# lxm0851/mp3

Measured on AMD Instinct MI355X. Metric: stereo MP3 frames/s (128 kbps 44.1 kHz) at 1/2/4/8 GPU; % HBM roofline, higher is better.
Workload: dtype f32; 1 GPU; C3: full Layer III decode (Huffman->PCM), 65536 streams x 32 frames per GPU per step; streams_per_gpu=65536, hz=44100, seed=default, parallelism=streams sharded, 1 process per GPU, no data-path collective

## Files before the change

mp3_amd/csrc/mp3d_huffman.hip:

```cpp
#include <algorithm>

#include "mp3d_huffman_dev.h"

namespace mp3d {

#define RANK_BINS 320
#define RANK_BLOCK 1024
#define RANK_PER 4
#define RANK_SEG (RANK_BLOCK * RANK_PER)
__global__ void __launch_bounds__(RANK_BLOCK) k_rank(const uint64_t *__restrict__ sideu, int n_units,
                                                     uint32_t *__restrict__ perm) {
    __shared__ uint32_t h[RANK_BINS];
    MP3D_LDS_ENTRY();
    const int tid = threadIdx.x, seg0 = blockIdx.x * RANK_SEG;
    for (int i = tid; i < RANK_BINS; i += RANK_BLOCK) h[i] = 0u;
    __syncthreads();
    uint32_t bin[RANK_PER], r[RANK_PER];
#pragma unroll
    for (int j = 0; j < RANK_PER; j++) {
        const int u = seg0 + j * RANK_BLOCK + tid;
        const uint32_t bv = u < n_units ? (uint32_t)(sideu[u] >> 43) & 0x1FFu : 0u;
        bin[j] = RANK_BINS - 1u - (bv < RANK_BINS ? bv : RANK_BINS - 1u);
        r[j] = u < n_units ? atomicAdd(&h[bin[j]], 1u) : 0u;
    }
    __syncthreads();
    if (tid < 64) {
        uint32_t c[5], sum = 0u;
#pragma unroll
        for (int k = 0; k < 5; k++) {
            c[k] = h[5 * tid + k];
            sum += c[k];
        }
        const uint32_t incl = wave_incl_scan(sum);
        uint32_t run = incl - sum;
#pragma unroll
        for (int k = 0; k < 5; k++) {
            h[5 * tid + k] = run;
            run += c[k];
        }
    }
    __syncthreads();
#pragma unroll
    for (int j = 0; j < RANK_PER; j++) {
        const int u = seg0 + j * RANK_BLOCK + tid;
        if (u < n_units) perm[seg0 + h[bin[j]] + r[j]] = (uint32_t)u;
    }
}

__global__ void __launch_bounds__(HUFF_BLOCK) k_huffman(const uint8_t *__restrict__ md, const uint64_t *__restrict__ md_off,
                                                        const FrameRec *__restrict__ rec,
                                                        const uint64_t *__restrict__ sideu,
                                                        const DevTables *__restrict__ tab, int16_t *__restrict__ is_buf,
                                                        UnitMeta *__restrict__ meta, int n_units, int F,
                                                        uint32_t *__restrict__ work, const uint32_t *__restrict__ perm) {
    __shared__ __attribute__((aligned(16))) uint16_t s_lut[MP3D_LUT_MAX];
    __shared__ __attribute__((aligned(16))) uint32_t s_bits[4 + HUFF_WAVES * (HUFF_CAPW + 4)];
    __shared__ uint32_t s_tsel[32];
    __shared__ uint16_t s_lbnd[9][24];
    __shared__ uint8_t s_slen[32];
    __shared__ uint32_t s_c1s[256];
    MP3D_LDS_ENTRY();
    huff_tables_lane(tab, s_lut, s_tsel, s_lbnd, s_slen);
    static_assert(HUFF_BLOCK >= 256, "s_c1s: one entry per thread");
    if (threadIdx.x < 256) {
        const uint32_t v = threadIdx.x >> 4, s4 = threadIdx.x & 15u;
        int q[4], j = 0;
#pragma unroll
        for (int i = 0; i < 4; i++) {
            const int bit = (int)(v >> (3 - i)) & 1;
            q[i] = bit && ((s4 >> (3 - j)) & 1u) ? -1 : bit;
            j += bit;
        }
        s_c1s[threadIdx.x] = (uint32_t)(uint8_t)q[2] | (uint32_t)(uint8_t)q[0] << 8 | (uint32_t)(uint8_t)q[3] << 16 |
                             (uint32_t)(uint8_t)q[1] << 24;
    }
    __syncthreads();
    const int lane = threadIdx.x & 63, wv = threadIdx.x >> 6;
    uint32_t *bits = s_bits + 4 + wv * (HUFF_CAPW + 4);
    const uint32_t qbase = tab->lut_hdr.base[MP3D_LUT_TABLES - 1];
    const int qb1 = tab->lut_hdr.bits1[MP3D_LUT_TABLES - 1];
    const uint32_t c1b_base = ((qbase + (1u << qb1) + 1u) & ~1u) + MP3D_C1B_OFF;
    for (;;) {
        uint32_t t = 0u;
        if (lane == 0) t = atomicAdd(work, 1u);
        const int ubase = 64 * (int)__builtin_amdgcn_readfirstlane(t);
        if (ubase >= n_units) break;
        {
            const int u = ubase + lane < n_units ? (int)perm[ubase + lane] : n_units;
            const int fr = u >> 2, gr = (u >> 1) & 1, ch = u & 1;
            bool valid = u < n_units;
            const uint64_t mdo = md_off[(valid ? fr : 0) / F];
            FrameRec r;
            uint64_t sq[4] = {0, 0, 0, 0};
            if (valid) {
                r = rec[fr];
                valid = r.frame_bytes && !(r.first_gr & (REC_TAG | REC_DROP)) && ch < r.nch && (gr == 0 || !r.lsf);
                const ulonglong2 a = *(const ulonglong2 *)&sideu[u & ~3];
                const ulonglong2 b = *(const ulonglong2 *)&sideu[(u & ~3) + 2];
                sq[0] = a.x; sq[1] = a.y; sq[2] = b.x; sq[3] = b.y;
            }
            const int first_gr = valid ? (r.first_gr & 3) : 0;
            const int nch = valid ? r.nch : 1;
            const bool dec = valid && gr >= first_gr;
            const int q = u & 3;
            const uint64_t side = sq[q];
            const uint32_t p23 = dec ? (uint32_t)(side >> 52) : 0u;
            uint32_t before = 0;
#pragma unroll
            for (int qq = 0; qq < 3; qq++)
                if (qq < q && (qq >> 1) >= first_gr && (qq & 1) < nch) before += (uint32_t)(sq[qq] >> 52);
            const uint32_t start = dec ? r.md_bit + before : 0u;
            const int scfsi_raw = (int)(side >> 1) & 15;
            const bool long_blk = !(((side >> 30) & 1) && ((side >> 28) & 3) == 2);
            const int scfsi = (gr == 1 && long_blk) ? scfsi_raw : 0;
            const bool need_g0 = dec && scfsi && first_gr == 0;
            const uint32_t g0_start = r.md_bit + (ch ? (uint32_t)(sq[0] >> 52) : 0u);
            const uint32_t lenA = need_g0 ? HUFF_G0W : 0u;
            const uint32_t w0 = start >> 5;
            const uint32_t dA = need_g0 ? w0 - (g0_start >> 5) : 0u;
            const uint32_t lenB = dec ? ((((start + p23 + 31) >> 5) + 2 - w0 + 3) & ~3u) : 0u;
            const uint32_t len = lenA + lenB;
            const uint32_t incl = wave_incl_scan(len);
            const uint32_t off = incl - len;
            const uint32_t *src = (const uint32_t *)(md + (dec ? mdo : 0)) + w0;

            bool pending = dec;
            while (__ballot(pending)) {
                const uint32_t base = wave_min(pending ? off : 0xFFFFFFFFu);
                const bool inb = pending && off + len - base <= HUFF_STAGEW;
                wave_sync();
                if (inb) {
                    uint32_t *dst = bits + (off - base);
                    for (uint32_t i = 0; i < len; i += 16) {
                        uint4 v[4];
#pragma unroll
                        for (int k = 0; k < 4; k++) {
                            const uint32_t q = i + 4 * k;
                            if (q < len) v[k] = *(const uint4 *)(src + (int)(q < lenA ? q - dA : q - lenA));
                        }
#pragma unroll
                        for (int k = 0; k < 4; k++)
                            if (i + 4 * k < len)
                                *(uint4 *)(dst + i + 4 * k) =
                                    make_uint4(bswap32(v[k].x), bswap32(v[k].y), bswap32(v[k].z), bswap32(v[k].w));
                    }
                }
                wave_sync();
                if (inb) {
                    const uint32_t seg = 32u * (off - base + lenA) - 32u * w0;
                    uint32_t pos = start + seg;
                    int lsf_pre = 0;
                    if (r.lsf) {
                        const uint32_t pp = read_sf_lsf((lds_cu32)bits, pos, side, (uint8_t *)&meta[u]);
                        pos = pp & 0x7FFFFFFFu;
                        lsf_pre = (int)(pp >> 31);
                    } else {
                        uint32_t sfw[10];
#pragma unroll
                        for (int i = 0; i < 10; i++) sfw[i] = 0u;
                        if (need_g0) {
                            read_sf(bits, g0_start + seg - 32u * (lenA - dA), sq[ch], 0, sfw, s_slen);
                        }
                        pos = read_sf(bits, pos, side, scfsi, sfw, s_slen);
                        uint8_t *mrec = (uint8_t *)&meta[u];
                        *(uint4 *)mrec = make_uint4(sfw[0], sfw[1], sfw[2], sfw[3]);
                        *(uint4 *)(mrec + 16) = make_uint4(sfw[4], sfw[5], sfw[6], sfw[7]);
                        *(uint2 *)(mrec + 32) = make_uint2(sfw[8], sfw[9]);
                    }
                    const int ws = (int)(side >> 30) & 1;
                    const int bv2 = 2 * ((int)(side >> 43) & 0x1FF);
                    int r1, r2;
                    uint32_t ts0, ts1, ts2;
                    if (ws) {
                        const bool sh = ((side >> 28) & 3) == 2;
                        r1 = r.sr_idx < 3 ? 36 : sh ? (r.sr_idx == 8 ? 72 : 36) : (r.sr_idx == 8 ? 108 : 54);
                        r2 = 576;
                        ts0 = s_tsel[(side >> 22) & 31];
                        ts1 = s_tsel[(side >> 17) & 31];
                        ts2 = ts1;
                    } else {
                        const int rc0 = (int)(side >> 11) & 15, rc1 = (int)(side >> 8) & 7;
                        const int b1 = rc0 + 1;
                        int b2 = rc0 + rc1 + 2;
                        if (b2 > 22) b2 = 22;
                        r1 = s_lbnd[r.sr_idx][b1];
                        r2 = s_lbnd[r.sr_idx][b2];
                        ts0 = s_tsel[(side >> 25) & 31];
                        ts1 = s_tsel[(side >> 20) & 31];
                        ts2 = s_tsel[(side >> 15) & 31];
                    }
                    r1 = r1 < bv2 ? r1 : bv2;
                    r2 = r2 < bv2 ? r2 : bv2;
                    int16_t *row = is_buf + (size_t)u * MP3D_IS_ROW;
                    int k = 0;
                    const uint32_t end_bit = start + seg + p23;
                    uint4 pend = make_uint4(0u, 0u, 0u, 0u);
                    bool held = false;
                    for (; __ballot(k < bv2); k += 8) {
                        uint32_t wv[4];
#pragma unroll
                        for (int j = 0; j < 4; j++) {
                            const int kk = k + 2 * j;
                            const uint32_t ts = kk < r1 ? ts0 : (kk < r2 ? ts1 : ts2);
                            const uint32_t tb = ts & 0xFFFFu, s1 = (ts >> 16) & 63u, lin = ts >> 24;
                            uint32_t hi, lo;
                            win64g(bits, pos, hi, lo);
                            const uint32_t i1 = tb + (hi >> s1);
                            const uint32_t e1 = s_lut[i1];
                            const uint32_t nb = __builtin_amdgcn_ubfe(e1, 11, 4);
                            uint32_t b11 = __builtin_amdgcn_ubfe(e1, 0, 11);
                            __asm__("" : "+v"(b11));
                            const uint32_t sub = (b11 << 2) + __builtin_amdgcn_ubfe(hi, s1 - nb, nb);
                            const uint32_t i2 = (e1 & 0x8000u) ? sub : i1;
                            const uint32_t e = s_lut[i2];
                            const uint32_t x = (e >> 4) & 15u, y = e & 15u, len_c = (e >> 8) & 31u;
                            const uint32_t sx = (e >> 13) & 1u, sy = (e >> 14) & 1u;
                            const uint32_t rb = shl64hi_a(hi, lo, len_c);
                            const uint32_t nx = x == 15u ? lin : 0u, ny = y == 15u ? lin : 0u;
                            const uint32_t t0 = 32u - nx, t1 = t0 - sx, t2 = t1 - ny, t3 = t2 - sy;
                            const uint32_t ex = __builtin_amdgcn_ubfe(rb, t0, nx);
                            const uint32_t ey = __builtin_amdgcn_ubfe(rb, t2, ny);
                            const int mx = __builtin_amdgcn_sbfe((int)rb, t1, 1u), my = __builtin_amdgcn_sbfe((int)rb, t3, 1u);
                            const bool live = kk < bv2 && pos < end_bit;
                            pos += live ? len_c + (32u - t3) : 0u;
                            const int X = ((int)(x + ex) ^ mx) - mx, Y = ((int)(y + ey) ^ my) - my;
                            wv[j] = live ? __builtin_amdgcn_perm((uint32_t)Y, (uint32_t)X, 0x05040100u) : 0u;
                        }
                        const uint4 cur = make_uint4(wv[0], wv[1], wv[2], wv[3]);
                        if (held) {
                            *(uint4 *)(row + k - 8) = pend;
                            *(uint4 *)(row + k) = cur;
                        } else {
                            pend = cur;
                        }
                        held = !held;
                    }
                    if (held) *(uint4 *)(row + k - 8) = pend;
                    k = bv2;
                    const bool c1b = (side >> 5) & 1;
                    const uint32_t c1base = c1b ? c1b_base : qbase, c1sh = c1b ? 28u : 32u - (uint32_t)qb1;
                    auto c1_store = [&](int kq, uint32_t se) {
                        *(uint2 *)(row + kq) = make_uint2(__builtin_amdgcn_perm(se, se, 0x09030801u),
                                                          __builtin_amdgcn_perm(se << 8, se, 0x0B070A05u));
                    };
                    auto c1_dec = [&](uint32_t hw, uint32_t &se, uint32_t &nb) {
                        const uint32_t e = s_lut[c1base + (hw >> c1sh)];
                        const uint32_t v = e & 15u, lq = (e >> 8) & 31u;
                        nb = lq + __builtin_popcount(v);
                        se = s_c1s[(v << 4) | ((hw << lq) >> 28)];
                    };
                    while (k <= 572 && pos < end_bit) {
                        const uint32_t hw = win32g(bits, pos);
                        uint32_t se0, n0, se1, n1;
                        c1_dec(hw, se0, n0);
                        if (pos + n0 > end_bit) break;
                        pos += n0;
                        bool two = k <= 568 && pos < end_bit;
                        if (two) {
                            c1_dec(hw << n0, se1, n1);
                            two = pos + n1 <= end_bit;
                        }
                        if (!two) {
                            c1_store(k, se0);
                            k += 4;
                            break;
                        }
                        pos += n1;
                        const uint4 q = make_uint4(
                            __builtin_amdgcn_perm(se0, se0, 0x09030801u), __builtin_amdgcn_perm(se0 << 8, se0, 0x0B070A05u),
                            __builtin_amdgcn_perm(se1, se1, 0x09030801u), __builtin_amdgcn_perm(se1 << 8, se1, 0x0B070A05u));
                        __builtin_memcpy(row + k, &q, 16);
                        k += 8;
                    }
                    const int nz_end = k;
                    UnitMeta m;
                    m.global_gain = (uint8_t)(side >> 35);
                    m.block_type = (uint8_t)(ws ? (side >> 28) & 3 : 0);
                    m.mixed = (uint8_t)(ws && ((side >> 28) & 3) == 2 ? (side >> 27) & 1 : 0);
                    m.scalefac_scale = (uint8_t)((side >> 6) & 1);
                    m.preflag = (uint8_t)(r.lsf ? lsf_pre : (int)((side >> 7) & 1));
                    m.sbg[0] = (uint8_t)(ws ? (side >> 14) & 7 : 0);
                    m.sbg[1] = (uint8_t)(ws ? (side >> 11) & 7 : 0);
                    m.sbg[2] = (uint8_t)(ws ? (side >> 8) & 7 : 0);
                    m.nz_end = (uint16_t)nz_end;
                    m.part2_3_length = (uint16_t)p23;
                    m.used_bits = (uint16_t)(pos - start - seg);
                    m.flags = (uint16_t)(r.lsf ? ((side >> 31) & 1) << 1 : 0);
                    *(uint4 *)((uint8_t *)&meta[u] + 40) = *(const uint4 *)((const uint8_t *)&m + 40);
                }
                pending = pending && !inb;
            }
            if (valid && !dec) {
                int16_t *out = is_buf + (size_t)u * MP3D_IS_ROW;
                for (int kk = 0; kk < 576; kk += 8) *(uint4 *)(out + kk) = make_uint4(0, 0, 0, 0);
                UnitMeta m;
#pragma unroll
                for (int i = 0; i < 10; i++) ((uint32_t *)m.sf)[i] = 0u;
                const int ws = (int)(side >> 30) & 1;
                m.global_gain = (uint8_t)(side >> 35);
                m.block_type = (uint8_t)(ws ? (side >> 28) & 3 : 0);
                m.mixed = (uint8_t)(ws && ((side >> 28) & 3) == 2 ? (side >> 27) & 1 : 0);
                m.scalefac_scale = (uint8_t)((side >> 6) & 1);
                m.preflag = (uint8_t)(r.lsf ? 0 : (int)((side >> 7) & 1));
                m.sbg[0] = (uint8_t)(ws ? (side >> 14) & 7 : 0);
                m.sbg[1] = (uint8_t)(ws ? (side >> 11) & 7 : 0);
                m.sbg[2] = (uint8_t)(ws ? (side >> 8) & 7 : 0);
                m.nz_end = 0;
                m.part2_3_length = 0;
                m.used_bits = 0;
                m.flags = (uint16_t)(1 | (r.lsf ? ((side >> 31) & 1) << 1 : 0));
                meta[u] = m;
            }
        }
    }
}

__global__ void __launch_bounds__(64 * HW_UNITS) k_huffman_wave(const uint8_t *__restrict__ md,
                                                              const uint64_t *__restrict__ md_off,
                                                              const FrameRec *__restrict__ rec,
                                                              const uint64_t *__restrict__ sideu,
                                                              const DevTables *__restrict__ tab,
                                                              int16_t *__restrict__ is_buf,
                                                              UnitMeta *__restrict__ meta, int n_units, int F) {
    __shared__ __attribute__((aligned(16))) uint16_t s_lut[MP3D_LUT_MAX];
    __shared__ __attribute__((aligned(16))) uint32_t s_bits[HW_UNITS][HW_WORDS + 4];
    __shared__ uint32_t s_tsel[32];
    __shared__ uint16_t s_lbnd[9][24];
    __shared__ uint8_t s_slen[32];
    MP3D_LDS_ENTRY();
    huff_tables<64 * HW_UNITS>(tab, s_lut, s_tsel, s_lbnd, s_slen, threadIdx.x);
    __syncthreads();
    const int lane = threadIdx.x & 63;
    const int wv = __builtin_amdgcn_readfirstlane((int)(threadIdx.x >> 6));
    const int u = blockIdx.x * HW_UNITS + wv;
    if (u >= n_units) return;
    huffman_wave_unit(md, md_off, rec, sideu, tab, is_buf, meta, F, u, lane, s_bits[wv], s_lut, s_tsel, s_lbnd, s_slen);
}

void launch_huffman(const uint8_t *md, const uint64_t *md_off, const FrameRec *rec, const uint64_t *sideu,
                    const DevTables *tab, int16_t *is_buf, UnitMeta *meta, int n_streams, int F, int n_cu, bool wave,
                    uint32_t *work, uint32_t *rank, hipStream_t strm) {
    int n_units = n_streams * F * 4;
    if (wave) {
        hipLaunchKernelGGL(k_huffman_wave, dim3((n_units + HW_UNITS - 1) / HW_UNITS), dim3(64 * HW_UNITS), 0, strm, md,
                           md_off, rec, sideu, tab, is_buf, meta, n_units, F);
        return;
    }
    const int rounds = (n_units + 63) / 64;
    int blocks = (rounds + HUFF_WAVES - 1) / HUFF_WAVES;
    const int cus = n_cu > 0 ? n_cu : 256;
    blocks = blocks < cus ? (blocks > 0 ? blocks : 1) : cus;
    (void)hipMemsetAsync(work, 0, sizeof(uint32_t), strm);
    hipLaunchKernelGGL(k_rank, dim3((n_units + RANK_SEG - 1) / RANK_SEG), dim3(RANK_BLOCK), 0, strm, sideu, n_units, rank);
    hipLaunchKernelGGL(k_huffman, dim3(blocks), dim3(HUFF_BLOCK), 0, strm, md, md_off, rec, sideu, tab, is_buf, meta,
                       n_units, F, work, (const uint32_t *)rank);
}

}
```

Measured before the change: 203.3 million frames/s.

## Reduce VGPR pressure in Huffman kernel and batch row stores in fours

Moves wave-uniform values (wave index, LUT base, table bits) into scalar registers via readfirstlane. Recomputes segment lengths and side-info fields inside the loop, using asm barriers to stop the compiler keeping them live. Also makes the staging loads unconditional by clamping the index. The big-value store loop now buffers four 16-byte groups before writing them together instead of two, which widens the stores but holds more registers.

```diff
diff --git a/mp3_amd/csrc/mp3d_huffman.hip b/mp3_amd/csrc/mp3d_huffman.hip
--- a/mp3_amd/csrc/mp3d_huffman.hip
+++ b/mp3_amd/csrc/mp3d_huffman.hip
@@ -75,12 +75,13 @@
                              (uint32_t)(uint8_t)q[1] << 24;
     }
     __syncthreads();
-    const int lane = threadIdx.x & 63, wv = threadIdx.x >> 6;
+    const int wv = __builtin_amdgcn_readfirstlane((int)(threadIdx.x >> 6));
     uint32_t *bits = s_bits + 4 + wv * (HUFF_CAPW + 4);
-    const uint32_t qbase = tab->lut_hdr.base[MP3D_LUT_TABLES - 1];
-    const int qb1 = tab->lut_hdr.bits1[MP3D_LUT_TABLES - 1];
+    const uint32_t qbase = (uint32_t)__builtin_amdgcn_readfirstlane((int)tab->lut_hdr.base[MP3D_LUT_TABLES - 1]);
+    const int qb1 = __builtin_amdgcn_readfirstlane((int)tab->lut_hdr.bits1[MP3D_LUT_TABLES - 1]);
     const uint32_t c1b_base = ((qbase + (1u << qb1) + 1u) & ~1u) + MP3D_C1B_OFF;
     for (;;) {
+        const int lane = lane_now();
         uint32_t t = 0u;
         if (lane == 0) t = atomicAdd(work, 1u);
         const int ubase = 64 * (int)__builtin_amdgcn_readfirstlane(t);
@@ -89,8 +90,10 @@
             const int u = ubase + lane < n_units ? (int)perm[ubase + lane] : n_units;
             const int fr = u >> 2, gr = (u >> 1) & 1, ch = u & 1;
             bool valid = u < n_units;
-            const uint64_t mdo = md_off[(valid ? fr : 0) / F];
-            FrameRec r;
+            int Fr = F;
+            __asm__ volatile("" : "+s"(Fr));
+            const uint64_t mdo = md_off[(valid ? fr : 0) / Fr];
+            FrameRec r = {};
             uint64_t sq[4] = {0, 0, 0, 0};
             if (valid) {
                 r = rec[fr];
@@ -115,17 +118,24 @@
             const int scfsi = (gr == 1 && long_blk) ? scfsi_raw : 0;
             const bool need_g0 = dec && scfsi && first_gr == 0;
             const uint32_t g0_start = r.md_bit + (ch ? (uint32_t)(sq[0] >> 52) : 0u);
-            const uint32_t lenA = need_g0 ? HUFF_G0W : 0u;
-            const uint32_t w0 = start >> 5;
-            const uint32_t dA = need_g0 ? w0 - (g0_start >> 5) : 0u;
-            const uint32_t lenB = dec ? ((((start + p23 + 31) >> 5) + 2 - w0 + 3) & ~3u) : 0u;
-            const uint32_t len = lenA + lenB;
-            const uint32_t incl = wave_incl_scan(len);
-            const uint32_t off = incl - len;
-            const uint32_t *src = (const uint32_t *)(md + (dec ? mdo : 0)) + w0;
+            uint32_t lenA, dA, w0;
+            auto seg_len = [&](uint32_t st, uint32_t g0s) {
+                lenA = need_g0 ? HUFF_G0W : 0u;
+                w0 = st >> 5;
+                dA = need_g0 ? w0 - (g0s >> 5) : 0u;
+                const uint32_t lenB = dec ? ((((st + p23 + 31) >> 5) + 2 - w0 + 3) & ~3u) : 0u;
+                return lenA + lenB;
+            };
+            const uint32_t len0 = seg_len(start, g0_start);
+            const uint32_t incl = wave_incl_scan(len0);
+            const uint32_t off = incl - len0;
 
             bool pending = dec;
             while (__ballot(pending)) {
+                uint32_t st = start, g0s = g0_start;
+                __asm__ volatile("" : "+v"(st), "+v"(g0s));
+                const uint32_t len = seg_len(st, g0s);
+                const uint32_t *src = (const uint32_t *)(md + (dec ? mdo : 0)) + w0;
                 const uint32_t base = wave_min(pending ? off : 0xFFFFFFFFu);
                 const bool inb = pending && off + len - base <= HUFF_STAGEW;
                 wave_sync();
@@ -135,9 +145,10 @@
                         uint4 v[4];
 #pragma unroll
                         for (int k = 0; k < 4; k++) {
-                            const uint32_t q = i + 4 * k;
-                            if (q < len) v[k] = *(const uint4 *)(src + (int)(q < lenA ? q - dA : q - lenA));
-                        }
+                            const uint32_t q = min(i + 4 * k, len - 4u);
+                            v[k] = *(const uint4 *)(src + (int)(q < lenA ? q - dA : q - lenA));
+                        }
+                        __asm__ volatile("" : "+v"(v[0].x), "+v"(v[1].x), "+v"(v[2].x), "+v"(v[3].x));
 #pragma unroll
                         for (int k = 0; k < 4; k++)
                             if (i + 4 * k < len)
@@ -159,9 +170,12 @@
 #pragma unroll
                         for (int i = 0; i < 10; i++) sfw[i] = 0u;
                         if (need_g0) {
-                            read_sf(bits, g0_start + seg - 32u * (lenA - dA), sq[ch], 0, sfw, s_slen);
-                        }
-                        pos = read_sf(bits, pos, side, scfsi, sfw, s_slen);
+                            read_sf(bits, g0_start + seg - 32u * (lenA - dA), sideu[(u & ~3) + ch], 0, sfw, s_slen);
+                        }
+                        uint32_t slo = (uint32_t)side;
+                        __asm__ volatile("" : "+v"(slo));
+                        const bool lb = !(((slo >> 30) & 1u) && ((slo >> 28) & 3u) == 2u);
+                        pos = read_sf(bits, pos, side, (gr == 1 && lb) ? (int)(slo >> 1) & 15 : 0, sfw, s_slen);
                         uint8_t *mrec = (uint8_t *)&meta[u];
                         *(uint4 *)mrec = make_uint4(sfw[0], sfw[1], sfw[2], sfw[3]);
                         *(uint4 *)(mrec + 16) = make_uint4(sfw[4], sfw[5], sfw[6], sfw[7]);
@@ -194,9 +208,7 @@
                     int16_t *row = is_buf + (size_t)u * MP3D_IS_ROW;
                     int k = 0;
                     const uint32_t end_bit = start + seg + p23;
-                    uint4 pend = make_uint4(0u, 0u, 0u, 0u);
-                    bool held = false;
-                    for (; __ballot(k < bv2); k += 8) {
+                    auto group = [&](int k) __attribute__((always_inline)) -> uint4 {
                         uint32_t wv[4];
 #pragma unroll
                         for (int j = 0; j < 4; j++) {
@@ -226,16 +238,35 @@
                             const int X = ((int)(x + ex) ^ mx) - mx, Y = ((int)(y + ey) ^ my) - my;
                             wv[j] = live ? __builtin_amdgcn_perm((uint32_t)Y, (uint32_t)X, 0x05040100u) : 0u;
                         }
-                        const uint4 cur = make_uint4(wv[0], wv[1], wv[2], wv[3]);
-                        if (held) {
-                            *(uint4 *)(row + k - 8) = pend;
-                            *(uint4 *)(row + k) = cur;
-                        } else {
-                            pend = cur;
-                        }
-                        held = !held;
-                    }
-                    if (held) *(uint4 *)(row + k - 8) = pend;
+                        return make_uint4(wv[0], wv[1], wv[2], wv[3]);
+                    };
+                    uint4 p0 = make_uint4(0u, 0u, 0u, 0u), p1 = p0, p2 = p0;
+                    int held = 0;
+                    for (;;) {
+                        if (!__ballot(k < bv2)) break;
+                        p0 = group(k);
+                        k += 8;
+                        held = 1;
+                        if (!__ballot(k < bv2)) break;
+                        p1 = group(k);
+                        k += 8;
+                        held = 2;
+                        if (!__ballot(k < bv2)) break;
+                        p2 = group(k);
+                        k += 8;
+                        held = 3;
+                        if (!__ballot(k < bv2)) break;
+                        const uint4 cur = group(k);
+                        *(uint4 *)(row + k - 24) = p0;
+                        *(uint4 *)(row + k - 16) = p1;
+                        *(uint4 *)(row + k - 8) = p2;
+                        *(uint4 *)(row + k) = cur;
+                        k += 8;
+                        held = 0;
+                    }
+                    if (held >= 1) *(uint4 *)(row + k - 8 * held) = p0;
+                    if (held >= 2) *(uint4 *)(row + k - 8 * held + 8) = p1;
+                    if (held >= 3) *(uint4 *)(row + k - 8) = p2;
                     k = bv2;
                     const bool c1b = (side >> 5) & 1;
                     const uint32_t c1base = c1b ? c1b_base : qbase, c1sh = c1b ? 28u : 32u - (uint32_t)qb1;
```

After: 199.5 million frames/s. -1.9%, worse.
